# akopich/spark-gp

Measured on AMD Instinct MI355X. Metric: rows/sec (full GP fit: BCM hyperopt + PPA), higher is better.
Workload: dtype fp32; 1 GPU; model=ARD-RBF GP regression, m=1000, expert=100, maxIter=100, restart=False, rows=10000000, dim=32, active_set=1000, expert_size=100, ppa_precision=mixed, parallelism=expert-parallel dp1

## Files before the change

### spark_gp_amd/ops/csrc/linalg_lds.h

```cpp
#pragma once
#include <hip/hip_runtime.h>
#include <math.h>

#ifndef WG
#define WG 512
#endif
#define NB 32

typedef __attribute__((ext_vector_type(4))) float mfma_f32x4_t;

__device__ inline double wave_sum(double v) {
#pragma unroll
  for (int off = 32; off; off >>= 1) v += __shfl_down(v, off, 64);
  return v;
}

__device__ inline double block_sum(double v, double* red, int tid) {
  v = wave_sum(v);
  if ((tid & 63) == 0) red[tid >> 6] = v;
  __syncthreads();
  if (tid == 0) {
    double s = 0;
#pragma unroll
    for (int w = 0; w < WG / 64; ++w) s += red[w];
    red[0] = s;
  }
  __syncthreads();
  double out = red[0];
  __syncthreads();
  return out;
}

__device__ inline float bcast_lane(float x, int src) {
  return __builtin_bit_cast(
      float, __builtin_amdgcn_readlane(__builtin_bit_cast(int, x), src));
}

__device__ inline void tri_decode(int f, int& a, int& b) {
  a = (int)((sqrtf(8.f * (float)f + 1.f) - 1.f) * 0.5f);
  while ((a + 1) * (a + 2) / 2 <= f) ++a;
  while (a * (a + 1) / 2 > f) --a;
  b = f - a * (a + 1) / 2;
}

__device__ inline float dotv(const float* p, const float* q, int c0,
                             int c1) {
  float s = 0.f;
  int c = c0;
  for (; c < c1 && (c & 3); ++c) s += p[c] * q[c];
  float4 a4 = {0.f, 0.f, 0.f, 0.f};
  for (; c + 3 < c1; c += 4) {
    const float4 a = *(const float4*)(p + c);
    const float4 b = *(const float4*)(q + c);
    a4.x += a.x * b.x;
    a4.y += a.y * b.y;
    a4.z += a.z * b.z;
    a4.w += a.w * b.w;
  }
  s += (a4.x + a4.y) + (a4.z + a4.w);
  for (; c < c1; ++c) s += p[c] * q[c];
  return s;
}

__device__ inline float dotm(const float* p, const float* q, int sq,
                             int c0, int c1) {
  float s = 0.f;
  int c = c0;
  for (; c < c1 && (c & 3); ++c) s += p[c] * q[c * sq];
  float s0 = 0.f, s1 = 0.f, s2 = 0.f, s3 = 0.f;
  for (; c + 3 < c1; c += 4) {
    const float4 a = *(const float4*)(p + c);
    s0 += a.x * q[c * sq];
    s1 += a.y * q[(c + 1) * sq];
    s2 += a.z * q[(c + 2) * sq];
    s3 += a.w * q[(c + 3) * sq];
  }
  s += (s0 + s1) + (s2 + s3);
  for (; c < c1; ++c) s += p[c] * q[c * sq];
  return s;
}

__device__ inline float dot4(const float* p, int sp, const float* q, int sq,
                             int c0, int c1) {
  float s0 = 0.f, s1 = 0.f, s2 = 0.f, s3 = 0.f;
  int c = c0;
  for (; c + 3 < c1; c += 4) {
    s0 += p[c * sp] * q[c * sq];
    s1 += p[(c + 1) * sp] * q[(c + 1) * sq];
    s2 += p[(c + 2) * sp] * q[(c + 2) * sq];
    s3 += p[(c + 3) * sp] * q[(c + 3) * sq];
  }
  for (; c < c1; ++c) s0 += p[c * sp] * q[c * sq];
  return (s0 + s1) + (s2 + s3);
}

__device__ inline void chol_invert_lower(float* Abuf, float* Tbuf,
                                         const int k, const int SA,
                                         const int tid_in, int* bad,
                                         double* misc,
                                         unsigned long long* jclk = nullptr) {
  int tid = tid_in;
  const int nblk = (k + NB - 1) / NB;
  for (int J = 0; J < nblk; ++J) {
    asm volatile("" : "+v"(tid));
    const int lane = tid & 63;
    const int jb = J * NB;
    const int bs = min(NB, k - jb);
    float* D = Abuf + (size_t)jb * SA + jb;
    const int pj = jb - NB;
    unsigned long long jt0 = 0, jt1 = 0;
    if (jclk && tid == 0) jt0 = wall_clock64();

    if (J > 0) {
      for (int f = tid; f < bs * bs; f += WG) {
        const int r = f / bs, c = f - r * bs;
        if (c > r) continue;
        const int i = jb + r, cc = jb + c;
        Abuf[(size_t)i * SA + cc] -=
            dotv(Abuf + (size_t)i * SA + pj,
                 Abuf + (size_t)cc * SA + pj, 0, NB);
      }
      __syncthreads();
    }
    if (jclk && (tid == 0 || tid == 64)) jt1 = wall_clock64();

    const int nq = (bs + 7) / 8;
    float* Vq = Tbuf;
    float* TS = Tbuf + 256;
    const int t0r = jb + bs;
    const int nrp = k - t0r;
    const int ntri_rest = nrp * (nrp + 1) / 2;
    for (int q = 0; q < nq; ++q) {
      const int qb = q * 8;
      const int sbs = min(8, bs - qb);
      if (tid < 64) {
        __builtin_amdgcn_s_setprio(1);
        {
          const int j = lane & 7;
          float row[8];
#pragma unroll
          for (int c = 0; c < 8; ++c)
            row[c] = (j < sbs && c < sbs && c <= j)
                         ? D[(size_t)(qb + j) * SA + qb + c]
                         : (c == j ? 1.f : 0.f);
          bool ok = true, nonfin = false;
          float mprod = 1.f;
          int expsum = 0;
          float myrs = 1.f;
          float rsv = 1.f;
#pragma unroll
          for (int ss = 0; ss < 8; ++ss) {
            float l[8];
#pragma unroll
            for (int c = 0; c < 8; ++c) l[c] = bcast_lane(row[ss], c);
            const float piv = l[ss];
            if (ss < sbs) {
              const bool fin = isfinite(piv);
              nonfin = nonfin || (ok && !fin);
              ok = ok && fin && (piv > 0.f);
              mprod *= __builtin_amdgcn_frexp_mantf(piv);
              expsum += __builtin_amdgcn_frexp_expf(piv);
            }
            const float rs = rsqrtf(piv);
            if (j == ss) myrs = rs;
            const float w = (j > ss) ? rs * row[ss] : 0.f;
#pragma unroll
            for (int c = ss + 1; c < 8; ++c) row[c] -= (rs * l[c]) * w;
          }
#pragma unroll
          for (int c = 0; c < 8; ++c) {
            rsv = bcast_lane(myrs, c);
            row[c] *= rsv;
          }
          if (lane < 8 && j < sbs) {
#pragma unroll
            for (int c = 0; c < 8; ++c)
              if (c <= j) D[(size_t)(qb + j) * SA + qb + c] = row[c];
          }
          float v[8];
#pragma unroll
          for (int i = 0; i < 8; ++i) v[i] = (i == j) ? myrs : 0.f;
#pragma unroll
          for (int i = 0; i < 8; ++i) {
            float rowi[8];
#pragma unroll
            for (int c = 0; c < 8; ++c) rowi[c] = bcast_lane(row[c], i);
            if (j < i) {
              float sacc = 0.f;
#pragma unroll
              for (int c = 0; c < 8; ++c)
                if (c >= j && c < i) sacc += rowi[c] * v[c];
              v[i] = -sacc * __builtin_amdgcn_rcpf(rowi[i]);
            }
          }
          if (lane < 8) {
#pragma unroll
            for (int i = 0; i < 8; ++i) Vq[q * 64 + i * 8 + j] = v[i];
          }
          if (lane == 0) {
            if (!ok) {
              if (*bad == 0) *bad = nonfin ? 2 : 1;
            } else {
              misc[0] += (double)__logf(mprod)
                         + (double)expsum * 0.6931471805599453;
            }
          }
        }
        __builtin_amdgcn_s_setprio(0);
      } else if (J > 0) {
        for (int f = (tid - 64) + q * (WG - 64); f < nrp * bs;
             f += (WG - 64) * nq) {
          const int r = f / bs, c = f - r * bs;
          const int i = t0r + r, cc = jb + c;
          Abuf[(size_t)i * SA + cc] -=
              dotv(Abuf + (size_t)i * SA + pj,
                   Abuf + (size_t)cc * SA + pj, 0, NB);
        }
        for (int f = (tid - 64) + q * (WG - 64); f < ntri_rest;
             f += (WG - 64) * nq) {
          int a, b;
          tri_decode(f, a, b);
          const int i = t0r + a, c = t0r + b;
          Abuf[(size_t)i * SA + c] -=
              dotv(Abuf + (size_t)i * SA + pj,
                   Abuf + (size_t)c * SA + pj, 0, NB);
        }
      }
      __syncthreads();
      if (*bad) break;
      const int p0 = qb + sbs;
      const int pr = bs - p0;
      if (pr > 0) {
        for (int f = tid; f < pr * 8; f += WG) {
          const int r = f >> 3, c = f & 7;
          if (c >= sbs) continue;
          float sacc = 0.f;
          const float* ar = D + (size_t)(p0 + r) * SA + qb;
          const float* vr = Vq + q * 64 + c * 8;
          for (int t = 0; t <= c; ++t) sacc += ar[t] * vr[t];
          TS[f] = sacc;
        }
        __syncthreads();
        for (int f = tid; f < pr * 8; f += WG) {
          const int r = f >> 3, c = f & 7;
          if (c >= sbs) continue;
          D[(size_t)(p0 + r) * SA + qb + c] = TS[f];
        }
        __syncthreads();
        const int ntri = pr * (pr + 1) / 2;
        for (int f = tid; f < ntri; f += WG) {
          int a, b;
          tri_decode(f, a, b);
          const int i = p0 + a, c = p0 + b;
          Abuf[(size_t)(jb + i) * SA + jb + c] -=
              dotv(D + (size_t)i * SA + qb, D + (size_t)c * SA + qb,
                   0, sbs);
        }
        __syncthreads();
      }
    }
    unsigned long long at0 = 0;
    if (jclk && tid == 0) {
      at0 = wall_clock64();
      jclk[2] += at0 - jt1;
    }
    if (*bad == 0) {
      for (int Jq = nq - 1; Jq >= 0; --Jq) {
        const int jb8 = Jq * 8;
        const int nblks = nq - 1 - Jq;
        for (int f = tid; f < nblks * 64; f += WG) {
          const int blk = f >> 6;
          const int ib = (Jq + 1 + blk) * 8;
          const int i = (f >> 3) & 7, j = f & 7;
          const int gi = ib + i;
          float u = 0.f;
          if (gi < bs && jb8 + j < bs) {
            u = dotm(D + (size_t)gi * SA, D + jb8 + j, SA,
                     jb8 + 8, min(gi + 1, bs));
          }
          TS[f] = u;
        }
        __syncthreads();
        for (int f = tid; f < nblks * 64; f += WG) {
          const int blk = f >> 6;
          const int ib = (Jq + 1 + blk) * 8;
          const int i = (f >> 3) & 7, j = f & 7;
          const int gi = ib + i;
          if (gi >= bs || jb8 + j >= bs) continue;
          float sacc = 0.f;
          const float* ts = TS + blk * 64 + i * 8;
          const float* vv = Vq + Jq * 64;
#pragma unroll
          for (int t = 0; t < 8; ++t) sacc += ts[t] * vv[t * 8 + j];
          D[(size_t)gi * SA + jb8 + j] = -sacc;
        }
        for (int f = tid; f < 64; f += WG) {
          const int i = (f >> 3) & 7, j = f & 7;
          const int gi = jb8 + i, gj = jb8 + j;
          if (gi < bs && gj <= gi) D[(size_t)gi * SA + gj] = Vq[Jq * 64 + f];
        }
        __syncthreads();
      }
    }
    if (jclk && tid == 0) jclk[3] += wall_clock64() - at0;
    __syncthreads();
    if (jclk && tid == 0) {
      const unsigned long long t2 = wall_clock64();
      jclk[0] += jt1 - jt0;
      jclk[1] += t2 - jt1;
      jt0 = t2;
    }
    if (*bad) break;

    const int t0 = jb + bs;
    const int nr = k - t0;
    if (nr > 0) {
      for (int f = tid; f < nr * bs; f += WG) {
        int r = f / bs, c = f - r * bs;
        Tbuf[r * 36 + c] = Abuf[(size_t)(t0 + r) * SA + jb + c];
      }
      __syncthreads();
      {
        const int w8 = tid >> 6;
        const int fl16 = lane & 15, fkg = lane >> 4;
        const int nti = (nr + 15) / 16, ntj = (bs + 15) / 16;
        for (int t = w8; t < nti * ntj; t += WG / 64) {
          const int ti = t / ntj, tj = t - ti * ntj;
          mfma_f32x4_t a = {0.f, 0.f, 0.f, 0.f};
          const int fr = ti * 16 + fl16;
          const int fc = tj * 16 + fl16;
          for (int c0 = 0; c0 < bs; c0 += 4) {
            const int tt = c0 + fkg;
            const float av = (fr < nr && tt < bs)
                                 ? Tbuf[fr * 36 + tt] : 0.f;
            const float bv = (fc < bs && tt <= fc)
                                 ? D[(size_t)fc * SA + tt] : 0.f;
            a = __builtin_amdgcn_mfma_f32_16x16x4f32(av, bv, a, 0, 0, 0);
          }
#pragma unroll
          for (int r = 0; r < 4; ++r) {
            const int gr = ti * 16 + fkg * 4 + r;
            const int gc = tj * 16 + fl16;
            if (gr < nr && gc < bs)
              Abuf[(size_t)(t0 + gr) * SA + jb + gc] = a[r];
          }
        }
      }
      __syncthreads();
    }
    if (jclk && tid == 0) jclk[4] += wall_clock64() - jt0;
  }

  if (*bad) return;
  unsigned long long dt0 = 0;
  if (jclk && tid == 0) dt0 = wall_clock64();
  for (int J = nblk - 2; J >= 0; --J) {
    asm volatile("" : "+v"(tid));
    const int lane = tid & 63;
    const int jb = J * NB;
    const int bs = NB;
    const int t0 = jb + bs;
    const int nr = k - t0;
    const int w8 = tid >> 6;
    const int fl16 = lane & 15, fkg = lane >> 4;
    const int nti = (nr + 15) / 16, ntj = (bs + 15) / 16;
    for (int t = w8; t < nti * ntj; t += WG / 64) {
      const int ti = t / ntj, tj = t - ti * ntj;
      mfma_f32x4_t a = {0.f, 0.f, 0.f, 0.f};
      const int fr = t0 + ti * 16 + fl16;
      const int fj = tj * 16 + fl16;
      for (int c0 = t0; c0 < k; c0 += 4) {
        const int cc = c0 + fkg;
        const float av = (fr < k && cc < k && cc <= fr)
                             ? Abuf[(size_t)fr * SA + cc] : 0.f;
        const float bv = (cc < k && fj < bs)
                             ? Abuf[(size_t)cc * SA + jb + fj] : 0.f;
        a = __builtin_amdgcn_mfma_f32_16x16x4f32(av, bv, a, 0, 0, 0);
      }
#pragma unroll
      for (int r = 0; r < 4; ++r) {
        const int gr = ti * 16 + fkg * 4 + r;
        const int gc = tj * 16 + fl16;
        if (gr < nr && gc < bs) Tbuf[gr * 36 + gc] = a[r];
      }
    }
    __syncthreads();
    for (int t = w8; t < nti * ntj; t += WG / 64) {
      const int ti = t / ntj, tj = t - ti * ntj;
      mfma_f32x4_t a = {0.f, 0.f, 0.f, 0.f};
      const int fr = ti * 16 + fl16;
      const int fj = tj * 16 + fl16;
      for (int c0 = 0; c0 < bs; c0 += 4) {
        const int tt = c0 + fkg;
        const float av = (fr < nr && tt < bs)
                             ? Tbuf[fr * 36 + tt] : 0.f;
        const float bv = (tt < bs && fj < bs && tt >= fj)
                             ? Abuf[(size_t)(jb + tt) * SA + jb + fj]
                             : 0.f;
        a = __builtin_amdgcn_mfma_f32_16x16x4f32(av, bv, a, 0, 0, 0);
      }
#pragma unroll
      for (int r = 0; r < 4; ++r) {
        const int gr = ti * 16 + fkg * 4 + r;
        const int gc = tj * 16 + fl16;
        if (gr < nr && gc < bs)
          Abuf[(size_t)(t0 + gr) * SA + jb + gc] = -a[r];
      }
    }
    __syncthreads();
  }
  if (jclk && tid == 0) jclk[5] += wall_clock64() - dt0;
}
```

Before: 24.53 million rows/s.

## Run diagonal-block factorization in a single wave with wave-level LDS sync

The per-8-column panel factorization and trailing update inside each 32-wide diagonal block now run entirely in wave 0, synchronized with wave-scope fences and waitcnt instead of block-wide barriers. The other waves do the off-diagonal trailing updates without per-q barriers. Removing the many __syncthreads per sub-block is meant to cut barrier overhead on the critical path. The triangle update is packed two elements per lane with an unfused dot to keep numerics close to before. The cost is that the diagonal work is serialized onto 64 lanes, and the single-wave LDS ordering is harder to get right.

```diff
diff --git a/spark_gp_amd/ops/csrc/linalg_lds.h b/spark_gp_amd/ops/csrc/linalg_lds.h
--- a/spark_gp_amd/ops/csrc/linalg_lds.h
+++ b/spark_gp_amd/ops/csrc/linalg_lds.h
@@ -62,6 +62,19 @@
   return s;
 }
 
+__device__ inline float dot8_unfused(const float* p, const float* q) {
+#pragma clang fp contract(off)
+  const float4 a0 = *(const float4*)p, b0 = *(const float4*)q;
+  const float4 a1 = *(const float4*)(p + 4), b1 = *(const float4*)(q + 4);
+  const float m0 = a0.x * b0.x, m1 = a0.y * b0.y;
+  const float m2 = a0.z * b0.z, m3 = a0.w * b0.w;
+  const float n0 = a1.x * b1.x, n1 = a1.y * b1.y;
+  const float n2 = a1.z * b1.z, n3 = a1.w * b1.w;
+  const float x = (0.f + m0) + n0, y = (0.f + m1) + n1;
+  const float z = (0.f + m2) + n2, w = (0.f + m3) + n3;
+  return 0.f + ((x + y) + (z + w));
+}
+
 __device__ inline float dotm(const float* p, const float* q, int sq,
                              int c0, int c1) {
   float s = 0.f;
@@ -92,6 +105,13 @@
   }
   for (; c < c1; ++c) s0 += p[c * sp] * q[c * sq];
   return (s0 + s1) + (s2 + s3);
+}
+
+__device__ inline void wave_lds_sync() {
+  __builtin_amdgcn_fence(__ATOMIC_RELEASE, "wavefront");
+  asm volatile("s_waitcnt lgkmcnt(0)" ::: "memory");
+  __builtin_amdgcn_wave_barrier();
+  __builtin_amdgcn_fence(__ATOMIC_ACQUIRE, "wavefront");
 }
 
 __device__ inline void chol_invert_lower(float* Abuf, float* Tbuf,
@@ -130,11 +150,12 @@
     const int t0r = jb + bs;
     const int nrp = k - t0r;
     const int ntri_rest = nrp * (nrp + 1) / 2;
-    for (int q = 0; q < nq; ++q) {
-      const int qb = q * 8;
-      const int sbs = min(8, bs - qb);
-      if (tid < 64) {
-        __builtin_amdgcn_s_setprio(1);
+    if (tid < 64) {
+      __builtin_amdgcn_s_setprio(1);
+      int w0ok = 1;
+      for (int q = 0; q < nq; ++q) {
+        const int qb = q * 8;
+        const int sbs = min(8, bs - qb);
         {
           const int j = lane & 7;
           float row[8];
@@ -197,6 +218,7 @@
 #pragma unroll
             for (int i = 0; i < 8; ++i) Vq[q * 64 + i * 8 + j] = v[i];
           }
+          w0ok = __builtin_amdgcn_readlane((int)ok, 0);
           if (lane == 0) {
             if (!ok) {
               if (*bad == 0) *bad = nonfin ? 2 : 1;
@@ -206,64 +228,79 @@
             }
           }
         }
-        __builtin_amdgcn_s_setprio(0);
-      } else if (J > 0) {
-        for (int f = (tid - 64) + q * (WG - 64); f < nrp * bs;
-             f += (WG - 64) * nq) {
-          const int r = f / bs, c = f - r * bs;
-          const int i = t0r + r, cc = jb + c;
-          Abuf[(size_t)i * SA + cc] -=
-              dotv(Abuf + (size_t)i * SA + pj,
-                   Abuf + (size_t)cc * SA + pj, 0, NB);
-        }
-        for (int f = (tid - 64) + q * (WG - 64); f < ntri_rest;
-             f += (WG - 64) * nq) {
-          int a, b;
-          tri_decode(f, a, b);
-          const int i = t0r + a, c = t0r + b;
-          Abuf[(size_t)i * SA + c] -=
-              dotv(Abuf + (size_t)i * SA + pj,
-                   Abuf + (size_t)c * SA + pj, 0, NB);
-        }
-      }
-      __syncthreads();
-      if (*bad) break;
-      const int p0 = qb + sbs;
-      const int pr = bs - p0;
-      if (pr > 0) {
-        for (int f = tid; f < pr * 8; f += WG) {
-          const int r = f >> 3, c = f & 7;
-          if (c >= sbs) continue;
-          float sacc = 0.f;
-          const float* ar = D + (size_t)(p0 + r) * SA + qb;
-          const float* vr = Vq + q * 64 + c * 8;
-          for (int t = 0; t <= c; ++t) sacc += ar[t] * vr[t];
-          TS[f] = sacc;
-        }
-        __syncthreads();
-        for (int f = tid; f < pr * 8; f += WG) {
-          const int r = f >> 3, c = f & 7;
-          if (c >= sbs) continue;
-          D[(size_t)(p0 + r) * SA + qb + c] = TS[f];
-        }
-        __syncthreads();
-        const int ntri = pr * (pr + 1) / 2;
-        for (int f = tid; f < ntri; f += WG) {
-          int a, b;
-          tri_decode(f, a, b);
-          const int i = p0 + a, c = p0 + b;
-          Abuf[(size_t)(jb + i) * SA + jb + c] -=
-              dotv(D + (size_t)i * SA + qb, D + (size_t)c * SA + qb,
-                   0, sbs);
-        }
-        __syncthreads();
-      }
-    }
-    unsigned long long at0 = 0;
-    if (jclk && tid == 0) {
-      at0 = wall_clock64();
-      jclk[2] += at0 - jt1;
-    }
+        if (!w0ok) break;
+        wave_lds_sync();
+        const int p0 = qb + sbs;
+        const int pr = bs - p0;
+        if (pr > 0) {
+          if (lane < pr) {
+            float* ap = D + (size_t)(p0 + lane) * SA + qb;
+            const float4 a0 = *(const float4*)ap;
+            const float4 a1 = *(const float4*)(ap + 4);
+            const float ar[8] = {a0.x, a0.y, a0.z, a0.w,
+                                 a1.x, a1.y, a1.z, a1.w};
+            const float* vr = Vq + q * 64;
+            float o[8];
+#pragma unroll
+            for (int c = 0; c < 8; ++c) {
+              float sacc = 0.f;
+#pragma unroll
+              for (int t = 0; t <= c; ++t)
+                sacc = __builtin_fmaf(ar[t], vr[c * 8 + t], sacc);
+              o[c] = sacc;
+            }
+            *(float4*)ap = make_float4(o[0], o[1], o[2], o[3]);
+            *(float4*)(ap + 4) = make_float4(o[4], o[5], o[6], o[7]);
+          }
+          wave_lds_sync();
+          const int wd = pr + 1, tot = ((pr + 1) >> 1) * wd;
+          const float rwd = 1.f / (float)wd;
+          for (int f0 = lane; f0 < tot; f0 += 128) {
+            float* tp[2];
+            const float *pa[2], *pb[2];
+            bool on[2];
+#pragma unroll
+            for (int u = 0; u < 2; ++u) {
+              const int f = f0 + 64 * u;
+              const int r = (int)(((float)f + 0.5f) * rwd);
+              const int c = f - r * wd;
+              const bool lo = c <= r;
+              on[u] = f < tot && (lo || pr - 1 - r != r);
+              const int a = on[u] ? (lo ? r : pr - 1 - r) : 0;
+              const int b = on[u] ? (lo ? c : c - r - 1) : 0;
+              tp[u] = D + (size_t)(p0 + a) * SA + p0 + b;
+              pa[u] = D + (size_t)(p0 + a) * SA + qb;
+              pb[u] = D + (size_t)(p0 + b) * SA + qb;
+            }
+            const float s0 = dot8_unfused(pa[0], pb[0]);
+            const float s1 = dot8_unfused(pa[1], pb[1]);
+            if (on[0]) *tp[0] -= s0;
+            if (on[1]) *tp[1] -= s1;
+          }
+          wave_lds_sync();
+        }
+      }
+      __builtin_amdgcn_s_setprio(0);
+      if (jclk && tid == 0) jclk[2] += wall_clock64() - jt1;
+    } else if (J > 0) {
+      for (int f = tid - 64; f < nrp * bs; f += WG - 64) {
+        const int r = f / bs, c = f - r * bs;
+        const int i = t0r + r, cc = jb + c;
+        Abuf[(size_t)i * SA + cc] -=
+            dotv(Abuf + (size_t)i * SA + pj,
+                 Abuf + (size_t)cc * SA + pj, 0, NB);
+      }
+      for (int f = tid - 64; f < ntri_rest; f += WG - 64) {
+        int a, b;
+        tri_decode(f, a, b);
+        const int i = t0r + a, c = t0r + b;
+        Abuf[(size_t)i * SA + c] -=
+            dotv(Abuf + (size_t)i * SA + pj,
+                 Abuf + (size_t)c * SA + pj, 0, NB);
+      }
+      if (jclk && tid == 64) jclk[3] += wall_clock64() - jt1;
+    }
+    __syncthreads();
     if (*bad == 0) {
       for (int Jq = nq - 1; Jq >= 0; --Jq) {
         const int jb8 = Jq * 8;
@@ -302,8 +339,6 @@
         __syncthreads();
       }
     }
-    if (jclk && tid == 0) jclk[3] += wall_clock64() - at0;
-    __syncthreads();
     if (jclk && tid == 0) {
       const unsigned long long t2 = wall_clock64();
       jclk[0] += jt1 - jt0;
```

Measured after the change: 25.25 million rows/s (median of 6 runs). +3.0%, better.
